# cassiePython/NeRF-Art

Hardware: AMD Instinct MI355X
Metric: rays/sec at 480x270x128spp VolSDF render (higher is better)
Workload: dtype pixels bf16x3 (sdf, nabla, radiance, compositing of the 192 final samples: f32 split into 2 bf16 terms, 3 MFMAs per product, f32 accumulate), Algorithm-1 sampler fp16x1 on error-compensated one-term weights (fp16 act x fp16 weight, 1 MFMA per product, f32 accumulate; model.calibrate_sampler()), guar

## Files before the change

### nerfart_amd/csrc/ray_common.h

```cpp
#pragma once
#include "nerfart_common.h"
#include "sample_cdf.h"
#include <math.h>

namespace nerfart {

__device__ __forceinline__ float wave_sum(float v) {
#pragma unroll
    for (int o = 32; o > 0; o >>= 1) v += __shfl_xor(v, o, 64);
    return v;
}
__device__ __forceinline__ float wave_max(float v) {
#pragma unroll
    for (int o = 32; o > 0; o >>= 1) v = fmaxf(v, __shfl_xor(v, o, 64));
    return v;
}
__device__ __forceinline__ float wave_excl_sum(float v) {
    const int lane = threadIdx.x & 63;
#pragma unroll
    for (int o = 1; o < 64; o <<= 1) {
        const float t = __shfl_up(v, o, 64);
        if (lane >= o) v += t;
    }
    const float e = __shfl_up(v, 1, 64);
// ... 82 lines not shown
            sR = __fmaf_rn(delta, sg, sR);
            sE = __fmaf_rn(t, x, sE);
        }
    }
    float R = wave_excl_sum(sR), E = wave_excl_sum(sE);
    float mx = -INFINITY;
#pragma unroll
    for (int i = 0; i < MAXSEG; ++i) {
        const int k = k0 + i;
        if (k < k1) {
            E = __fmaf_rn(c_t[i], c_x[i], E);
            float b = expf(-R) * (expf(E) - 1.f);
            if (isnan(b)) b = INFINITY;
            if (clamp) b = fminf(fmaxf(b, 0.f), 1e5f);
            if (w_out) w_out[k] = b;
            mx = fmaxf(mx, b);
            R = __fmaf_rn(c_delta[i], c_sigma[i], R);
        }
    }
    return wave_max(mx);
}

template <int MAXSEG>
struct SegConsts { float delta[MAXSEG], s[MAXSEG], dstar[MAXSEG], dd[MAXSEG]; int cnt; };

template <int MAXSEG>
__device__ __forceinline__ void load_seg_consts(const float* d, const float* s, int n, SegConsts<MAXSEG>& C) {
    const int lane = threadIdx.x & 63;
    const int nint = n - 1;
    const int seg = (nint + 63) >> 6;
    const int k0 = lane * seg;
    const int k1 = (k0 + seg < nint) ? k0 + seg : nint;
    C.cnt = k1 - k0;
    float dk = 0.f, sk = 0.f;
    if (k0 < k1) { dk = d[k0]; sk = s[k0]; }
#pragma unroll
    for (int i = 0; i < MAXSEG; ++i) {
        C.delta[i] = 0.f; C.s[i] = 0.f; C.dstar[i] = 0.f; C.dd[i] = 0.f;
        if (i < C.cnt) {
            const float dn = d[k0 + i + 1], sn = s[k0 + i + 1];
            const float delta = dn - dk;
            C.delta[i] = delta;
            C.s[i] = sk;
            C.dstar[i] = fmaxf(0.5f * (fabsf(sk) + fabsf(sn) - delta), 0.f);
            C.dd[i] = delta * delta;
            dk = dn; sk = sn;
        }
    }
}

template <int MAXSEG>
__device__ __forceinline__ float scan_consts(const SegConsts<MAXSEG>& C, float alpha, float beta) {
    const float a4b = alpha / (4.f * beta);
    float c_sigma[MAXSEG], c_t[MAXSEG], c_x[MAXSEG];
    float sR = 0.f, sE = 0.f;
#pragma unroll
    for (int i = 0; i < MAXSEG; ++i) {
        c_sigma[i] = 0.f; c_t[i] = 0.f; c_x[i] = 0.f;
        if (i < C.cnt) {
            const float sg = sdf_to_sigma(C.s[i], alpha, beta);
            const float t = a4b * C.dd[i];
            const float x = expf(-C.dstar[i] / beta);
            c_sigma[i] = sg; c_t[i] = t; c_x[i] = x;
            sR = __fmaf_rn(C.delta[i], sg, sR);
            sE = __fmaf_rn(t, x, sE);
        }
    }
    float R = wave_excl_sum(sR), E = wave_excl_sum(sE);
    float mx = -INFINITY;
#pragma unroll
    for (int i = 0; i < MAXSEG; ++i) {
        if (i < C.cnt) {
            E = __fmaf_rn(c_t[i], c_x[i], E);
            float b = expf(-R) * (expf(E) - 1.f);
            if (isnan(b)) b = INFINITY;
            mx = fmaxf(mx, b);
            R = __fmaf_rn(C.delta[i], c_sigma[i], R);
        }
    }
    return wave_max(mx);
}

__device__ __forceinline__ float error_bound_scan(const float* d, const float* s, int n, float alpha, float beta,
                                                  float* w_out, bool clamp) {
#ifndef NERFART_SCAN_GENERIC
    const int seg = (n - 1 + 63) >> 6;
    if (seg <= 8) return error_bound_scan_cached<8>(d, s, n, alpha, beta, w_out, clamp);
    if (seg <= 16) return error_bound_scan_cached<16>(d, s, n, alpha, beta, w_out, clamp);
    if (seg <= 24) return error_bound_scan_cached<24>(d, s, n, alpha, beta, w_out, clamp);
#endif
    return error_bound_scan_generic(d, s, n, alpha, beta, w_out, clamp);
}

__device__ __forceinline__ void opacity_cdf(const float* d, const float* s, int n, float alpha, float beta, float* cdf) {
    const int lane = threadIdx.x & 63;
    const int nint = n - 1;
    const int seg = (nint + 63) >> 6;
    const int k0 = lane * seg;
    const int k1 = (k0 + seg < nint) ? k0 + seg : nint;
    float sR = 0.f;
    for (int k = k0; k < k1; ++k) sR += sdf_to_sigma(s[k], alpha, beta) * (d[k + 1] - d[k]);
    float R = wave_excl_sum(sR);
    if (lane == 0) cdf[0] = 0.f;
    for (int k = k0; k < k1; ++k) {
        cdf[k + 1] = 1.f - expf(-R);
        R += sdf_to_sigma(s[k], alpha, beta) * (d[k + 1] - d[k]);
    }
}

__device__ __forceinline__ void bitonic_sort(float* a, int n) {
    const int lane = threadIdx.x & 63;
    for (int k = 2; k <= n; k <<= 1) {
        for (int j = k >> 1; j > 0; j >>= 1) {
            __syncthreads();
// ... 15 lines not shown
```

### nerfart_amd/csrc/volsdf_render.hip

```cpp
#include "ray_common.h"
#include "host_util.h"
#include <cstdlib>

namespace nerfart {

struct SamplerParams {
    int n;
    int cap;
    int n_up;
    int n_final;
    int max_bisect;
    int it;
    float eps;
    float alpha_net, beta_net;
    int u_final_stride;
    float guard;
    int* esc_list;
    int* esc_count;
};

__device__ __forceinline__ bool in_guard_band(const SamplerParams& P, float mx) {
    return P.guard > 0.f && fabsf(mx - P.eps) <= P.guard * P.eps;
}
__device__ __forceinline__ void escalate(const SamplerParams& P, int ray) {
// ... 8 lines not shown
    const int r = (int)(i / n), k = (int)(i - (long long)r * n);
    const float nr = near ? near[r] : near_s, fr = far ? far[r] : far_s;
    const float tk = t[k];
    out[(size_t)r * stride + k] = __fadd_rn(__fmul_rn(nr, __fsub_rn(1.f, tk)), __fmul_rn(fr, tk));
}

__global__ void k_normalize_dirs(const float* __restrict__ in, float* __restrict__ out, int n) {
    const int i = blockIdx.x * blockDim.x + threadIdx.x;
    if (i >= n) return;
    const float x = in[3 * i], y = in[3 * i + 1], z = in[3 * i + 2];
    const float nrm = fmaxf(sqrtf(x * x + y * y + z * z), 1e-12f);
    out[3 * i] = x / nrm; out[3 * i + 1] = y / nrm; out[3 * i + 2] = z / nrm;
}

__device__ __forceinline__ void load_row(float* dst, const float* src, int n) {
    for (int i = threadIdx.x; i < n; i += 64) dst[i] = src[i];
}

__device__ __forceinline__ void emit_final_samples(const float* d, const float* cdf, int n, const float* u_final,
                                                   int n_final, float* out) {
    for (int j = threadIdx.x; j < n_final; j += 64) out[j] = invert_cdf_at(d, cdf, n, u_final[j]);
}

__global__ void __launch_bounds__(64)
k_first_check(SamplerParams P, const float* __restrict__ dA, const float* __restrict__ sA,
              const float* __restrict__ u_final, float beta_plus0_denom, const float* __restrict__ far,
              float far_s, float* __restrict__ d_fine, float* __restrict__ beta_plus, float* __restrict__ beta_map,
              float* __restrict__ iter_usage, int* __restrict__ act_out, int* __restrict__ act_count) {
    extern __shared__ __attribute__((aligned(16))) float sm[];
    const int ray = blockIdx.x;
    float* d = sm; float* s = sm + P.n; float* cdf = sm + 2 * P.n;
    load_row(d, dA + (size_t)ray * P.cap, P.n);
    load_row(s, sA + (size_t)ray * P.cap, P.n);
    __syncthreads();
    const float mx = error_bound_scan(d, s, P.n, P.alpha_net, P.beta_net, nullptr, false);
    const float fr = far ? far[ray] : far_s;
    if (in_guard_band(P, mx)) { escalate(P, ray); return; }
    if (!(mx > P.eps)) {
        opacity_cdf(d, s, P.n, P.alpha_net, P.beta_net, cdf);
        __syncthreads();
        emit_final_samples(d, cdf, P.n, u_final + (size_t)ray * P.u_final_stride, P.n_final, d_fine + (size_t)ray * P.n_final);
        if (threadIdx.x == 0) { iter_usage[ray] = 0.f; beta_map[ray] = P.beta_net; }
    } else if (threadIdx.x == 0) {
        beta_plus[ray] = sqrtf((fr * fr) / beta_plus0_denom);
        act_out[atomicAdd(act_count, 1)] = ray;
    }
}

__global__ void __launch_bounds__(64)
k_upsample(SamplerParams P, const float* __restrict__ dA, const float* __restrict__ sA,
           const int* __restrict__ act, const float* __restrict__ beta_plus, const float* __restrict__ u_up,
           int clamp_bounds, int always_sort, float* __restrict__ d_new) {
    extern __shared__ __attribute__((aligned(16))) float sm[];
    const int slot = blockIdx.x, ray = act[slot];
    const int n = P.n;
    float* d = sm; float* s = sm + n; float* cdf = sm + 2 * n; float* w = sm + 3 * n; float* out = sm + 4 * n;
    load_row(d, dA + (size_t)ray * P.cap, n);
    load_row(s, sA + (size_t)ray * P.cap, n);
    __syncthreads();
    const float bp = beta_plus[ray];
    error_bound_scan(d, s, n, 1.f / bp, bp, w, clamp_bounds != 0);
    __syncthreads();
    const int lane = threadIdx.x;
    const int nint = n - 1, seg = (nint + 63) >> 6, k0 = lane * seg, k1 = (k0 + seg < nint) ? k0 + seg : nint;
    float part = 0.f;
    for (int k = k0; k < k1; ++k) { const float wk = w[k] + 1e-5f; w[k] = wk; part += wk; }
    const float total = wave_sum(part);
    float ps = 0.f;
    for (int k = k0; k < k1; ++k) ps += w[k] / total;
    float run = wave_excl_sum(ps);
    if (lane == 0) cdf[0] = 0.f;
    for (int k = k0; k < k1; ++k) { run += w[k] / total; cdf[k + 1] = run; }
    __syncthreads();
    for (int j = lane; j < P.n_up; j += 64) out[j] = invert_cdf_at(d, cdf, n, u_up[j + 1]);
    __syncthreads();
    if (always_sort || !__all((int)lane_row_in_order(out, P.n_up, lane))) bitonic_sort(out, P.n_up);
    for (int j = lane; j < P.n_up; j += 64) d_new[(size_t)slot * P.n_up + j] = out[j];
}

template <int MAXSEG>
__device__ __forceinline__ void merge_check_tail(const SamplerParams& P, int ray, const float* d, const float* s, float* cdf, int nm,
                                                 const float* __restrict__ u_final, float* __restrict__ d_fine, float* __restrict__ beta_plus,
                                                 float* __restrict__ beta_map, float* __restrict__ iter_usage, int* __restrict__ act_out,
                                                 int* __restrict__ act_count) {
    constexpr int NS = MAXSEG > 0 ? MAXSEG : 1;
    SegConsts<NS> C;
    if constexpr (MAXSEG > 0) load_seg_consts<NS>(d, s, nm, C);
    auto scan = [&](float alpha, float beta) -> float {
        if constexpr (MAXSEG > 0) return scan_consts<NS>(C, alpha, beta);
        else return error_bound_scan(d, s, nm, alpha, beta, nullptr, false);
    };
    const float mx = scan(P.alpha_net, P.beta_net);
    if (in_guard_band(P, mx)) { escalate(P, ray); return; }
    if (!(mx > P.eps)) {
        opacity_cdf(d, s, nm, P.alpha_net, P.beta_net, cdf);
        __syncthreads();
        emit_final_samples(d, cdf, nm, u_final + (size_t)ray * P.u_final_stride, P.n_final, d_fine + (size_t)ray * P.n_final);
        if (threadIdx.x == 0) { iter_usage[ray] = (float)P.it; beta_map[ray] = P.beta_net; }
    } else {
        float hi = beta_plus[ray], lo = P.beta_net;
        for (int b = 0; b < P.max_bisect; ++b) {
            const float mid = 0.5f * (lo + hi);
            const float m = scan(1.f / mid, mid);
            if (m <= P.eps) hi = mid; else lo = mid;
        }
        if (threadIdx.x == 0) {
            beta_plus[ray] = hi;
            act_out[atomicAdd(act_count, 1)] = ray;
        }
    }
}

__global__ void __launch_bounds__(64)
k_merge_check(SamplerParams P, const float* __restrict__ dA, const float* __restrict__ sA,
              float* __restrict__ dB, float* __restrict__ sB, const int* __restrict__ act,
              const float* __restrict__ d_new, const float* __restrict__ s_new, const float* __restrict__ u_final,
              float* __restrict__ d_fine, float* __restrict__ beta_plus, float* __restrict__ beta_map,
              float* __restrict__ iter_usage, int* __restrict__ act_out, int* __restrict__ act_count) {
    extern __shared__ __attribute__((aligned(16))) float sm[];
    const int slot = blockIdx.x, ray = act[slot];
    const int n = P.n, nu = P.n_up, nm = n + nu;
    float* d_old = sm; float* dn = sm + n;
    float* d = dn + nu; float* s = d + nm;
    const float* s_old = sA + (size_t)ray * P.cap;
    const float* sn = s_new + (size_t)slot * nu;
    load_row(d_old, dA + (size_t)ray * P.cap, n);
    load_row(dn, d_new + (size_t)slot * nu, nu);
    __syncthreads();
    for (int i = threadIdx.x; i < n; i += 64) {
        const int r = i + lower_bound(dn, nu, d_old[i]);
        d[r] = d_old[i]; s[r] = s_old[i];
    }
    for (int k = threadIdx.x; k < nu; k += 64) {
        const int r = k + upper_bound(d_old, n, dn[k]);
        d[r] = dn[k]; s[r] = sn[k];
    }
    __syncthreads();
    for (int i = threadIdx.x; i < nm; i += 64) {
        dB[(size_t)ray * P.cap + i] = d[i];
        sB[(size_t)ray * P.cap + i] = s[i];
    }
#ifndef NERFART_SCAN_GENERIC
    const int seg = (nm - 1 + 63) >> 6;
    if (seg <= 16) { merge_check_tail<16>(P, ray, d, s, d_old, nm, u_final, d_fine, beta_plus, beta_map, iter_usage, act_out, act_count); return; }
    if (seg <= 24) { merge_check_tail<24>(P, ray, d, s, d_old, nm, u_final, d_fine, beta_plus, beta_map, iter_usage, act_out, act_count); return; }
#endif
    merge_check_tail<0>(P, ray, d, s, d_old, nm, u_final, d_fine, beta_plus, beta_map, iter_usage, act_out, act_count);
}

__global__ void __launch_bounds__(64)
k_finalize_unconverged(SamplerParams P, const float* __restrict__ dA, const float* __restrict__ sA,
                       const int* __restrict__ act, const float* __restrict__ u_final,
                       const float* __restrict__ beta_plus, float* __restrict__ d_fine,
                       float* __restrict__ beta_map, float* __restrict__ iter_usage) {
    extern __shared__ __attribute__((aligned(16))) float sm[];
    const int ray = act[blockIdx.x];
    const int n = P.n;
    float* d = sm; float* s = sm + n; float* cdf = sm + 2 * n;
    load_row(d, dA + (size_t)ray * P.cap, n);
    load_row(s, sA + (size_t)ray * P.cap, n);
    __syncthreads();
    const float bp = beta_plus[ray];
    opacity_cdf(d, s, n, 1.f / bp, bp, cdf);
    __syncthreads();
    emit_final_samples(d, cdf, n, u_final + (size_t)ray * P.u_final_stride, P.n_final, d_fine + (size_t)ray * P.n_final);
    if (threadIdx.x == 0) { iter_usage[ray] = -1.f; beta_map[ray] = bp; }
}

__global__ void __launch_bounds__(64)
k_sort_concat(const float* __restrict__ a, int na, int a_stride, const float* __restrict__ b, int nb, int b_stride,
// ... 85 lines not shown
                                  float* __restrict__ beta_map, float* __restrict__ iter_usage) {
    const int slot = blockIdx.x, ray = list[slot], t = threadIdx.x;
    if (slot >= n) return;
    for (int j = t; j < n_final; j += 64) d_fine[(size_t)ray * n_final + j] = c_d_fine[(size_t)slot * n_final + j];
    if (t == 0) { beta_map[ray] = c_beta[slot]; iter_usage[ray] = c_iter[slot]; }
}

enum { SKIP_SEG = 32 };
constexpr float SKIP_THETA = 128.0f;

__global__ void k_live_init(int c0, int n, int* __restrict__ live, float* __restrict__ osum) {
    const int i = blockIdx.x * blockDim.x + threadIdx.x;
    if (i < n) { live[i] = c0 + i; osum[c0 + i] = 0.f; }
}

__global__ void k_gather_segment_depths(const int* __restrict__ live, int n_live, int P, int e0, int len, const float* __restrict__ d_all,
                                        float* __restrict__ c_d) {
    const long long i = (long long)blockIdx.x * blockDim.x + threadIdx.x;
    if (i >= (long long)n_live * len) return;
    const int slot = (int)(i / len), j = (int)(i - (long long)slot * len);
    c_d[i] = d_all[(size_t)live[slot] * P + e0 + j];
}

__global__ void k_scatter_segment(const int* __restrict__ live, int n_live, int P, int e0, int len, const float* __restrict__ c_sdf,
                                  const float* __restrict__ c_nabla, const float* __restrict__ c_rad, float* __restrict__ sdf,
                                  float* __restrict__ nabla, float* __restrict__ rad) {
    const long long i = (long long)blockIdx.x * blockDim.x + threadIdx.x;
    if (i >= (long long)n_live * len) return;
    const int slot = (int)(i / len), j = (int)(i - (long long)slot * len);
    const size_t q = (size_t)live[slot] * P + e0 + j;
    sdf[q] = c_sdf[i];
#pragma unroll
    for (int c = 0; c < 3; ++c) { nabla[3 * q + c] = c_nabla[3 * (size_t)i + c]; rad[3 * q + c] = c_rad[3 * (size_t)i + c]; }
}

__global__ void __launch_bounds__(256)
k_advance_live(const int* __restrict__ live, int n_live, int P, int e0, int len, const float* __restrict__ d_all, float alpha, float beta,
               float* __restrict__ osum, int* __restrict__ alive, float* sdf, float* __restrict__ nabla, float* __restrict__ rad) {
    const int slot = blockIdx.x * 4 + (threadIdx.x >> 6), lane = threadIdx.x & 63;
    if (slot >= n_live) return;
    const int ray = live[slot];
    const float* dr = d_all + (size_t)ray * P;
    const float* sr = sdf + (size_t)ray * P;
    float x = 0.f;
    if (lane < len) {
        const int k = e0 + lane;
        x = fmaxf(sdf_to_sigma(sr[k], alpha, beta) * (dr[k + 1] - dr[k]), 0.f);
    }
    float sum = osum[ray];
    for (int j = 0; j < len; ++j) sum = __fadd_rn(sum, __shfl(x, j, 64));
    const bool dead = sum >= SKIP_THETA;
    if (lane == 0) { osum[ray] = sum; alive[slot] = dead ? 0 : 1; }
    if (dead) {
        const size_t q0 = (size_t)ray * P + e0 + len;
        const int n = P - (e0 + len);
        for (int i = lane; i < n; i += 64) sdf[q0 + i] = 0.f;
        for (int i = lane; i < 3 * n; i += 64) { nabla[3 * q0 + i] = 0.f; rad[3 * q0 + i] = 0.f; }
    }
}

__global__ void __launch_bounds__(1024)
k_compact_live(const int* __restrict__ live, const int* __restrict__ alive, int n_live, int* __restrict__ live_next, int* __restrict__ n_next) {
    __shared__ int wsum[16];
    __shared__ int base_sh;
    const int t = threadIdx.x, lane = t & 63, wv = t >> 6;
    const int first = blockIdx.x * 1024;
    int part = 0;
    for (int i = t; i < first; i += 1024) part += alive[i];
#pragma unroll
    for (int o = 32; o > 0; o >>= 1) part += __shfl_xor(part, o, 64);
    if (lane == 0) wsum[wv] = part;
    __syncthreads();
    if (t == 0) { int b = 0; for (int w = 0; w < 16; ++w) b += wsum[w]; base_sh = b; }
    __syncthreads();
    const int base = base_sh;
    const int slot = first + t;
    const bool keep = slot < n_live && alive[slot] != 0;
// ... 37 lines not shown
    NERFART_HIP(hipGetLastError());
    return 0;
}

static int check_rows(const char* who, int n, int cap, int n_extra) {
    char msg[160];
    if (n < 2 || n > cap) snprintf(msg, sizeof(msg), "%s: needs 2 <= n <= cap (n = %d, cap = %d)", who, n, cap);
    else if ((long long)n + n_extra > cap) snprintf(msg, sizeof(msg), "%s: n + n_up = %lld exceeds the row capacity cap = %d", who, (long long)n + n_extra, cap);
    else return 0;
    set_last_error(msg);
    return 2;
}

static const char kLdsRefusal[] = "per-ray kernel needs more than 160 KiB of LDS (too many samples per ray)";

static int first_check_launch(int n_rays, int n, int cap, int n_final, float eps, float alpha_net, float beta_net,
                              const float* dA, const float* sA, const float* u_final, int u_final_stride,
                              float beta_plus0_denom, const float* far, float far_s, float* d_fine, float* beta_plus,
                              float* beta_map, float* iter_usage, int* act_out, int* act_count, float guard, int* esc_list, int* esc_count,
                              void* stream) {
    if (n_rays <= 0) return 0;
    SamplerParams P{n, cap, 0, n_final, 0, 0, eps, alpha_net, beta_net, u_final_stride, guard, esc_list, esc_count};
    const size_t lds = (size_t)3 * n * sizeof(float);
    if (int rc = set_lds((const void*)k_first_check, lds, kLdsRefusal)) return rc;
    hipLaunchKernelGGL(k_first_check, dim3(n_rays), dim3(64), lds, (hipStream_t)stream, P, dA, sA, u_final,
                       beta_plus0_denom, far, far_s, d_fine, beta_plus, beta_map, iter_usage, act_out, act_count);
    NERFART_HIP(hipGetLastError());
    return 0;
}

int nerfart_volsdf_first_check(int n_rays, int n, int cap, int n_final, float eps, float alpha_net, float beta_net,
                               const float* dA, const float* sA, const float* u_final, int u_final_stride,
                               float beta_plus0_denom, const float* far, float far_s, float* d_fine, float* beta_plus,
                               float* beta_map, float* iter_usage, int* act_out, int* act_count, void* stream) {
    if (n_rays <= 0) return 0;
    if (int rc = check_rows("volsdf_first_check", n, cap, 0)) return rc;
    return first_check_launch(n_rays, n, cap, n_final, eps, alpha_net, beta_net, dA, sA, u_final, u_final_stride, beta_plus0_denom, far, far_s, d_fine,
                              beta_plus, beta_map, iter_usage, act_out, act_count, 0.f, nullptr, nullptr, stream);
}

static int upsample_launch(int n_active, int n, int cap, int n_up, const float* dA, const float* sA, const int* act,
                           const float* beta_plus, const float* u_up, int clamp_bounds, float* d_new, void* stream) {
    if (n_active <= 0) return 0;
    if (n_up & (n_up - 1)) { set_last_error("n_up must be a power of two"); return 2; }
    SamplerParams P{n, cap, n_up, 0, 0, 0, 0.f, 0.f, 0.f};
    const size_t lds = ((size_t)4 * n + n_up) * sizeof(float);
    if (int rc = set_lds((const void*)k_upsample, lds, kLdsRefusal)) return rc;
    const char* e = std::getenv("NERFART_UPSAMPLE_SORT");
    const int always_sort = (e != nullptr && e[0] == 'a') ? 1 : 0;
    hipLaunchKernelGGL(k_upsample, dim3(n_active), dim3(64), lds, (hipStream_t)stream, P, dA, sA, act, beta_plus, u_up,
                       clamp_bounds, always_sort, d_new);
    NERFART_HIP(hipGetLastError());
    return 0;
}

int nerfart_volsdf_upsample(int n_active, int n, int cap, int n_up, const float* dA, const float* sA, const int* act,
                            const float* beta_plus, const float* u_up, int clamp_bounds, float* d_new, void* stream) {
    if (n_active <= 0) return 0;
    if (int rc = check_rows("volsdf_upsample", n, cap, 0)) return rc;
    return upsample_launch(n_active, n, cap, n_up, dA, sA, act, beta_plus, u_up, clamp_bounds, d_new, stream);
}

static int merge_check_launch(int n_active, int n, int cap, int n_up, int n_final, int max_bisect, int it, float eps,
                              float alpha_net, float beta_net, const float* dA, const float* sA, float* dB, float* sB,
                              const int* act, const float* d_new, const float* s_new, const float* u_final,
                              int u_final_stride, float* d_fine, float* beta_plus, float* beta_map, float* iter_usage,
                              int* act_out, int* act_count, float guard, int* esc_list, int* esc_count, void* stream) {
    if (n_active <= 0) return 0;
    SamplerParams P{n, cap, n_up, n_final, max_bisect, it, eps, alpha_net, beta_net, u_final_stride, guard, esc_list, esc_count};
    const size_t lds = ((size_t)3 * n + 3 * n_up) * sizeof(float);
    if (int rc = set_lds((const void*)k_merge_check, lds, kLdsRefusal)) return rc;
    hipLaunchKernelGGL(k_merge_check, dim3(n_active), dim3(64), lds, (hipStream_t)stream, P, dA, sA, dB, sB, act, d_new,
                       s_new, u_final, d_fine, beta_plus, beta_map, iter_usage, act_out, act_count);
    NERFART_HIP(hipGetLastError());
    return 0;
}

int nerfart_volsdf_merge_check(int n_active, int n, int cap, int n_up, int n_final, int max_bisect, int it, float eps,
                               float alpha_net, float beta_net, const float* dA, const float* sA, float* dB, float* sB,
                               const int* act, const float* d_new, const float* s_new, const float* u_final,
                               int u_final_stride, float* d_fine, float* beta_plus, float* beta_map, float* iter_usage,
                               int* act_out, int* act_count, void* stream) {
    if (n_active <= 0) return 0;
    if (int rc = check_rows("volsdf_merge_check", n, cap, n_up)) return rc;
    return merge_check_launch(n_active, n, cap, n_up, n_final, max_bisect, it, eps, alpha_net, beta_net, dA, sA, dB, sB, act, d_new, s_new, u_final,
                              u_final_stride, d_fine, beta_plus, beta_map, iter_usage, act_out, act_count, 0.f, nullptr, nullptr, stream);
}

static int finalize_launch(int n_active, int n, int cap, int n_final, const float* dA, const float* sA, const int* act,
                           const float* u_final, int u_final_stride, const float* beta_plus, float* d_fine,
                           float* beta_map, float* iter_usage, void* stream) {
    if (n_active <= 0) return 0;
    SamplerParams P{n, cap, 0, n_final, 0, 0, 0.f, 0.f, 0.f, u_final_stride};
    const size_t lds = (size_t)3 * n * sizeof(float);
    if (int rc = set_lds((const void*)k_finalize_unconverged, lds, kLdsRefusal)) return rc;
// ... 105 lines not shown
    if (!own_tables) {
        w.t_init = const_cast<float*>(t_init_dev); w.u_up = const_cast<float*>(u_up_dev); w.u_final = const_cast<float*>(u_final_dev);
    } else {
        if (int rc = upload_linspace_tables({{w.t_init, n_init}, {w.u_up, n_up + 2}, {w.u_final, n_final}}, stream)) return rc;
        if (u_final_per_ray) w.u_final = const_cast<float*>(u_final_dev);
    }
    if (int rc = nerfart_linspace_depths(w.t_init, n_init, near, far, near_s, far_s, n_rays, w.dA, cap, stream)) return rc;
    if (int rc = nerfart_sdf_fwd_rays(surf_blob, precision, rays_o, rays_dn, nullptr, w.dA, n_rays, n_init, cap, R_bg, w.sA, cap, stream)) return rc;
    NERFART_HIP(hipMemsetAsync(w.count, 0, COUNT_SLOTS * sizeof(int), stream));
    const float denom = (float)(4.0 * (double)(n_init - 1) * log(1.0 + (double)eps));
    if (int rc = first_check_launch(n_rays, n_init, cap, n_final, eps, alpha_net, beta_net, w.dA, w.sA, w.u_final,
                                    u_stride, denom, far, far_s, d_fine, w.beta_plus, beta_map, iter_usage, w.act0,
                                    w.count, guard, w.esc_list, w.count + ESC_SLOT, stream)) return rc;
    int h_count[COUNT_SLOTS];
    NERFART_HIP(hipMemcpyAsync(h_count, w.count, sizeof(h_count), hipMemcpyDeviceToHost, stream));
    NERFART_HIP(hipStreamSynchronize(stream));
    int n_act = h_count[0];
    float *dA = w.dA, *sA = w.sA, *dB = w.dB, *sB = w.sB;
    int *act = w.act0, *act_next = w.act1;
    int n = n_init;
    for (int it = 1; it <= max_iter && n_act > 0; ++it) {
        if (int rc = upsample_launch(n_act, n, cap, n_up, dA, sA, act, w.beta_plus, w.u_up, it > 1, w.d_new, stream)) return rc;
        if (int rc = nerfart_sdf_fwd_rays(surf_blob, precision, rays_o, rays_dn, act, w.d_new, n_act, n_up, n_up, R_bg, w.s_new, n_up, stream)) return rc;
        if (int rc = merge_check_launch(n_act, n, cap, n_up, n_final, max_bisect, it, eps, alpha_net, beta_net, dA, sA,
                                        dB, sB, act, w.d_new, w.s_new, w.u_final, u_stride, d_fine, w.beta_plus,
                                        beta_map, iter_usage, act_next, w.count + it, guard, w.esc_list, w.count + ESC_SLOT, stream)) return rc;
        NERFART_HIP(hipMemcpyAsync(h_count, w.count, sizeof(h_count), hipMemcpyDeviceToHost, stream));
        NERFART_HIP(hipStreamSynchronize(stream));
        n_act = h_count[it];
        float* t;
        t = dA; dA = dB; dB = t;
        t = sA; sA = sB; sB = t;
        int* ti = act; act = act_next; act_next = ti;
        n += n_up;
        if (guarded && late_round > 0 && it >= late_round) break;
    }
    if (!guarded) {
        if (n_act > 0)
            if (int rc = finalize_launch(n_act, n, cap, n_final, dA, sA, act, w.u_final, u_stride, w.beta_plus, d_fine,
                                         beta_map, iter_usage, stream)) return rc;
        return 0;
    }
    int n_esc = h_count[ESC_SLOT];
    if (n_act > 0) {
        NERFART_HIP(hipMemcpyAsync(w.esc_list + n_esc, act, sizeof(int) * (size_t)n_act, hipMemcpyDeviceToDevice, stream));
        n_esc += n_act;
    }
    if (n_escalated) *n_escalated = n_esc;
    if (n_esc == 0) return 0;
    hipLaunchKernelGGL(k_gather_rays, dim3(n_esc), dim3(64), 0, stream, w.esc_list, n_esc, rays_o, rays_dn, near, far,
                       u_final_per_ray ? u_final_dev : (const float*)nullptr, n_final, w.c_o, w.c_dn, w.c_near, w.c_far, w.c_u);
    NERFART_HIP(hipGetLastError());
    const float* u2 = u_final_per_ray ? w.c_u : (own_tables ? nullptr : u_final_dev);
    const int* esc_list = w.esc_list;
    float *c_d_fine = w.c_d_fine, *c_beta = w.c_beta, *c_iter = w.c_iter;
    profile_class0_as(4);
    const int rc_esc = fine_sample_run(esc_blob, esc_precision, nullptr, 0, 0.f, 0, w.c_o, w.c_dn, n_esc, near ? w.c_near : nullptr, far ? w.c_far : nullptr,
                                       near_s, far_s, R_bg, alpha_net, beta_net, eps, n_init, n_up, n_final, max_iter, max_bisect,
// ... 32 lines not shown

int nerfart_volsdf_fine_sample_guarded(const float* surf_blob, int precision, const float* esc_blob, int esc_precision, float guard,
                                       const float* rays_o, const float* rays_dn, int n_rays,
                                       const float* near, const float* far, float near_s, float far_s, float R_bg,
                                       float alpha_net, float beta_net, float eps, int n_init, int n_up, int n_final,
                                       int max_iter, int max_bisect, const float* t_init_dev, const float* u_up_dev,
                                       const float* u_final_dev, int u_final_per_ray, float* d_fine, float* beta_map,
                                       float* iter_usage, int* n_escalated, void* workspace, long long workspace_bytes, void* stream) {
    return nerfart_volsdf_fine_sample_guarded2(surf_blob, precision, esc_blob, esc_precision, guard, 0, rays_o, rays_dn, n_rays, near, far, near_s, far_s, R_bg,
                                               alpha_net, beta_net, eps, n_init, n_up, n_final, max_iter, max_bisect, t_init_dev, u_up_dev, u_final_dev,
                                               u_final_per_ray, d_fine, beta_map, iter_usage, n_escalated, workspace, workspace_bytes, stream);
}

typedef struct {
    float *rays_dn, *d_fine, *d_coarse, *t_coarse, *d_all, *sdf, *nabla, *rad, *beta_map, *iter_usage, *h7;
    char* sampler;
    size_t sampler_bytes;
    char* nabla_ws;
    size_t nabla_ws_bytes;
} render_ws_t;

typedef struct {
    int *live0, *live1, *alive, *n_live;
    float *osum, *c_depth, *c_sdf, *c_nabla, *c_rad;
} skip_ws_t;

static skip_ws_t carve_skip(Carver& c, int R, int P, int G) {
    skip_ws_t k;
    const size_t gpts = (size_t)G * (P < SKIP_SEG ? P : SKIP_SEG);
    k.live0 = c.take<int>((size_t)G);
    k.live1 = c.take<int>((size_t)G);
    k.alive = c.take<int>((size_t)G);
    k.n_live = c.take<int>(1);
    k.osum = c.take<float>((size_t)R);
    k.c_depth = c.take<float>(gpts);
    k.c_sdf = c.take<float>(gpts);
    k.c_nabla = c.take<float>(gpts * 3);
    k.c_rad = c.take<float>(gpts * 3);
    return k;
}

static int skip_group_rays(int R, int P, int k3_rays, size_t room) {
    const long long rk = k3_rays < R ? k3_rays : R;
    long long g = rk * P / (P < SKIP_SEG ? P : SKIP_SEG);
    if (g > R) g = R;
    for (; g > 1; g /= 2) {
        Carver c(nullptr);
        carve_skip(c, R, P, (int)g);
        if (c.off <= room) break;
    }
    return (int)g;
}

static render_ws_t carve_render(Carver& c, int R, int n_samples, int n_imp, int max_iter, int k3_rays) {
    render_ws_t w;
    const int P = n_samples + n_imp;
    const int n_init = 4 * n_samples, n_up = 4 * n_samples;
    w.rays_dn = c.take<float>((size_t)R * 3);
    w.d_fine = c.take<float>((size_t)R * n_imp);
    w.d_coarse = c.take<float>((size_t)R * n_samples);
    w.t_coarse = c.take<float>((size_t)n_samples);
    w.d_all = c.take<float>((size_t)R * P);
    w.sdf = c.take<float>((size_t)R * P);
    w.nabla = c.take<float>((size_t)R * P * 3);
    w.rad = c.take<float>((size_t)R * P * 3);
    w.beta_map = c.take<float>((size_t)R);
    w.iter_usage = c.take<float>((size_t)R);
    const int rk = k3_rays < R ? k3_rays : R;
    w.h7 = c.take<float>((size_t)rk * P * 256);
    w.sampler_bytes = sampler_bytes(R, n_init + max_iter * n_up, n_up, n_init, n_imp);
    w.sampler = c.take<char>(w.sampler_bytes);
    const long long nb0 = nerfart_sdf_nabla_workspace_bytes(0), nb1 = nerfart_sdf_nabla_workspace_bytes(1);
    w.nabla_ws_bytes = (size_t)(nb0 > nb1 ? nb0 : nb1);
    w.nabla_ws = c.take<char>(w.nabla_ws_bytes);
    return w;
}

long long nerfart_volsdf_render_workspace_bytes(int n_rays, int n_samples, int n_importance, int max_upsample_steps,
                                                int k3_rays_chunk) {
    Carver c(nullptr);
    carve_render(c, n_rays, n_samples, n_importance, max_upsample_steps, k3_rays_chunk);
    return (long long)c.off;
}

static int final_stage_skipping(const render_ws_t& w, const float* surf_blob, int precision, const float* rad_blob, int rad_precision, int view_tiles,
                                const float* rays_o, int n_rays, int P, float R_bg, float alpha, float beta, const float* d_all, float* sdf,
                                float* nabla, float* rad, int k3_rays, hipStream_t stream) {
    const int G = skip_group_rays(n_rays, P, k3_rays, w.sampler_bytes);
    Carver carver(w.sampler);
    const skip_ws_t k = carve_skip(carver, n_rays, P, G);
    if (carver.off > w.sampler_bytes) { set_last_error("render: workspace too small"); return 2; }
    int *live = k.live0, *live_next = k.live1;
    for (int c0 = 0; c0 < n_rays; c0 += G) {
        int n_live = (n_rays - c0 < G) ? n_rays - c0 : G;
        hipLaunchKernelGGL(k_live_init, dim3((n_live + 255) / 256), dim3(256), 0, stream, c0, n_live, live, k.osum);
        NERFART_HIP(hipGetLastError());
        for (int e0 = 0; e0 < P && n_live > 0; e0 += SKIP_SEG) {
            const int len = (P - e0 < SKIP_SEG) ? P - e0 : SKIP_SEG;
            const unsigned nb = (unsigned)(((long long)n_live * len + 255) / 256);
            hipLaunchKernelGGL(k_gather_segment_depths, dim3(nb), dim3(256), 0, stream, live, n_live, P, e0, len, d_all, k.c_depth);
            NERFART_HIP(hipGetLastError());
            if (int rc = nerfart_sdf_nabla_fwd_rays(surf_blob, precision, rays_o, w.rays_dn, live, k.c_depth, n_live, len, len, R_bg, k.c_sdf, k.c_nabla,
                                                    w.h7, w.nabla_ws, (long long)w.nabla_ws_bytes, stream)) return rc;
            if (int rc = nerfart_radiance_fwd_rays(rad_blob, rad_precision, view_tiles, rays_o, w.rays_dn, live, k.c_depth, n_live, len, len, k.c_nabla,
                                                   w.h7, k.c_rad, stream)) return rc;
            hipLaunchKernelGGL(k_scatter_segment, dim3(nb), dim3(256), 0, stream, live, n_live, P, e0, len, k.c_sdf, k.c_nabla, k.c_rad, sdf, nabla, rad);
            NERFART_HIP(hipGetLastError());
            if (e0 + len >= P) break;
            hipLaunchKernelGGL(k_advance_live, dim3((n_live + 3) / 4), dim3(256), 0, stream, live, n_live, P, e0, len, d_all, alpha, beta, k.osum,
                               k.alive, sdf, nabla, rad);
            NERFART_HIP(hipGetLastError());
            hipLaunchKernelGGL(k_compact_live, dim3((n_live + 1023) / 1024), dim3(1024), 0, stream, live, k.alive, n_live, live_next, k.n_live);
            NERFART_HIP(hipGetLastError());
            NERFART_HIP(hipMemcpyAsync(&n_live, k.n_live, sizeof(int), hipMemcpyDeviceToHost, stream));
            NERFART_HIP(hipStreamSynchronize(stream));
            int* t = live; live = live_next; live_next = t;
        }
    }
    return 0;
}

int nerfart_volsdf_render_staged2_fwd(const float* surf_blob, int precision, const float* rad_blob, int rad_precision, const float* sampler_blob,
                                     int sampler_precision, float sampler_guard, int sampler_late_round, int view_tiles, const float* rays_o,
                              const float* rays_d, int n_rays, float near_s, float far_s, float R_bg, float alpha,
                              float beta, float eps, int n_samples, int n_importance, int max_upsample_steps,
                              int max_bisection_steps, int white_bkgd, int k3_rays_chunk, const float* t_coarse_dev,
                              const float* t_init_dev, const float* u_up_dev, const float* u_final_dev, int u_final_per_ray,
                              float* rgb, float* depth, float* acc, float* normals, float* d_all_out, float* sdf_out, float* nabla_out,
                              float* radiance_out, float* sigma_out, float* p_out, float* tau_out, float* beta_map_out,
                              float* iter_usage_out, int* n_escalated, void* workspace, long long workspace_bytes, void* stream_) {
    hipStream_t stream = (hipStream_t)stream_;
    if (n_rays <= 0) return 0;
    if (!sampler_blob) { set_last_error("render: sampler_blob is NULL"); return 2; }
    if (n_samples < 2 || n_importance < 1 || k3_rays_chunk < 1) { set_last_error("render: bad sample counts"); return 2; }
// ... 89 lines not shown
```

Before: 344,200.

## Specialize sampler scans at launch, trim LDS rows, fuse scatter/advance, own h7 scratch

```diff
diff --git a/nerfart_amd/csrc/ray_common.h b/nerfart_amd/csrc/ray_common.h
--- a/nerfart_amd/csrc/ray_common.h
+++ b/nerfart_amd/csrc/ray_common.h
@@ -128,7 +128,7 @@
 }
 
 template <int MAXSEG>
-struct SegConsts { float delta[MAXSEG], s[MAXSEG], dstar[MAXSEG], dd[MAXSEG]; int cnt; };
+struct SegConsts { float delta[MAXSEG], s[MAXSEG], dstar[MAXSEG]; int cnt; };
 
 template <int MAXSEG>
 __device__ __forceinline__ void load_seg_consts(const float* d, const float* s, int n, SegConsts<MAXSEG>& C) {
@@ -142,32 +142,36 @@
     if (k0 < k1) { dk = d[k0]; sk = s[k0]; }
 #pragma unroll
     for (int i = 0; i < MAXSEG; ++i) {
-        C.delta[i] = 0.f; C.s[i] = 0.f; C.dstar[i] = 0.f; C.dd[i] = 0.f;
+        C.delta[i] = 0.f; C.s[i] = 0.f; C.dstar[i] = 0.f;
         if (i < C.cnt) {
             const float dn = d[k0 + i + 1], sn = s[k0 + i + 1];
             const float delta = dn - dk;
             C.delta[i] = delta;
             C.s[i] = sk;
             C.dstar[i] = fmaxf(0.5f * (fabsf(sk) + fabsf(sn) - delta), 0.f);
-            C.dd[i] = delta * delta;
             dk = dn; sk = sn;
         }
     }
+}
+
+__device__ __forceinline__ float squared_here(float v) {
+    asm volatile("" : "+v"(v));
+    return v * v;
 }
 
 template <int MAXSEG>
 __device__ __forceinline__ float scan_consts(const SegConsts<MAXSEG>& C, float alpha, float beta) {
     const float a4b = alpha / (4.f * beta);
-    float c_sigma[MAXSEG], c_t[MAXSEG], c_x[MAXSEG];
+    float c_sigma[MAXSEG], c_x[MAXSEG];
     float sR = 0.f, sE = 0.f;
 #pragma unroll
     for (int i = 0; i < MAXSEG; ++i) {
-        c_sigma[i] = 0.f; c_t[i] = 0.f; c_x[i] = 0.f;
+        c_sigma[i] = 0.f; c_x[i] = 0.f;
         if (i < C.cnt) {
             const float sg = sdf_to_sigma(C.s[i], alpha, beta);
-            const float t = a4b * C.dd[i];
+            const float t = a4b * squared_here(C.delta[i]);
             const float x = expf(-C.dstar[i] / beta);
-            c_sigma[i] = sg; c_t[i] = t; c_x[i] = x;
+            c_sigma[i] = sg; c_x[i] = x;
             sR = __fmaf_rn(C.delta[i], sg, sR);
             sE = __fmaf_rn(t, x, sE);
         }
@@ -177,7 +181,7 @@
 #pragma unroll
     for (int i = 0; i < MAXSEG; ++i) {
         if (i < C.cnt) {
-            E = __fmaf_rn(c_t[i], c_x[i], E);
+            E = __fmaf_rn(a4b * squared_here(C.delta[i]), c_x[i], E);
             float b = expf(-R) * (expf(E) - 1.f);
             if (isnan(b)) b = INFINITY;
             mx = fmaxf(mx, b);
@@ -187,15 +191,22 @@
     return wave_max(mx);
 }
 
+inline int scan_maxseg(int n) {
+#ifndef NERFART_SCAN_GENERIC
+    const int seg = (n - 1 + 63) >> 6;
+    if (seg <= 8) return 8;
+    if (seg <= 16) return 16;
+    if (seg <= 24) return 24;
+#endif
+    (void)n;
+    return 0;
+}
+
+template <int MAXSEG>
 __device__ __forceinline__ float error_bound_scan(const float* d, const float* s, int n, float alpha, float beta,
                                                   float* w_out, bool clamp) {
-#ifndef NERFART_SCAN_GENERIC
-    const int seg = (n - 1 + 63) >> 6;
-    if (seg <= 8) return error_bound_scan_cached<8>(d, s, n, alpha, beta, w_out, clamp);
-    if (seg <= 16) return error_bound_scan_cached<16>(d, s, n, alpha, beta, w_out, clamp);
-    if (seg <= 24) return error_bound_scan_cached<24>(d, s, n, alpha, beta, w_out, clamp);
-#endif
-    return error_bound_scan_generic(d, s, n, alpha, beta, w_out, clamp);
+    if constexpr (MAXSEG > 0) return error_bound_scan_cached<MAXSEG>(d, s, n, alpha, beta, w_out, clamp);
+    else return error_bound_scan_generic(d, s, n, alpha, beta, w_out, clamp);
 }
 
 __device__ __forceinline__ void opacity_cdf(const float* d, const float* s, int n, float alpha, float beta, float* cdf) {
diff --git a/nerfart_amd/csrc/volsdf_render.hip b/nerfart_amd/csrc/volsdf_render.hip
--- a/nerfart_amd/csrc/volsdf_render.hip
+++ b/nerfart_amd/csrc/volsdf_render.hip
@@ -54,6 +54,7 @@
     for (int j = threadIdx.x; j < n_final; j += 64) out[j] = invert_cdf_at(d, cdf, n, u_final[j]);
 }
 
+template <int MAXSEG>
 __global__ void __launch_bounds__(64)
 k_first_check(SamplerParams P, const float* __restrict__ dA, const float* __restrict__ sA,
               const float* __restrict__ u_final, float beta_plus0_denom, const float* __restrict__ far,
@@ -65,7 +66,7 @@
     load_row(d, dA + (size_t)ray * P.cap, P.n);
     load_row(s, sA + (size_t)ray * P.cap, P.n);
     __syncthreads();
-    const float mx = error_bound_scan(d, s, P.n, P.alpha_net, P.beta_net, nullptr, false);
+    const float mx = error_bound_scan<MAXSEG>(d, s, P.n, P.alpha_net, P.beta_net, nullptr, false);
     const float fr = far ? far[ray] : far_s;
     if (in_guard_band(P, mx)) { escalate(P, ray); return; }
     if (!(mx > P.eps)) {
@@ -79,6 +80,7 @@
     }
 }
 
+template <int MAXSEG, bool S_IN_LDS>
 __global__ void __launch_bounds__(64)
 k_upsample(SamplerParams P, const float* __restrict__ dA, const float* __restrict__ sA,
            const int* __restrict__ act, const float* __restrict__ beta_plus, const float* __restrict__ u_up,
@@ -86,12 +88,13 @@
     extern __shared__ __attribute__((aligned(16))) float sm[];
     const int slot = blockIdx.x, ray = act[slot];
     const int n = P.n;
-    float* d = sm; float* s = sm + n; float* cdf = sm + 2 * n; float* w = sm + 3 * n; float* out = sm + 4 * n;
+    float* d = sm; float* cdf = sm + n; float* w = sm + 2 * n; float* out = sm + 3 * n;
+    const float* s = sA + (size_t)ray * P.cap;
     load_row(d, dA + (size_t)ray * P.cap, n);
-    load_row(s, sA + (size_t)ray * P.cap, n);
+    if constexpr (S_IN_LDS) { float* sl = out + P.n_up; load_row(sl, s, n); s = sl; }
     __syncthreads();
     const float bp = beta_plus[ray];
-    error_bound_scan(d, s, n, 1.f / bp, bp, w, clamp_bounds != 0);
+    error_bound_scan<MAXSEG>(d, s, n, 1.f / bp, bp, w, clamp_bounds != 0);
     __syncthreads();
     const int lane = threadIdx.x;
     const int nint = n - 1, seg = (nint + 63) >> 6, k0 = lane * seg, k1 = (k0 + seg < nint) ? k0 + seg : nint;
@@ -110,24 +113,33 @@
     for (int j = lane; j < P.n_up; j += 64) d_new[(size_t)slot * P.n_up + j] = out[j];
 }
 
-template <int MAXSEG>
-__device__ __forceinline__ void merge_check_tail(const SamplerParams& P, int ray, const float* d, const float* s, float* cdf, int nm,
+template <int MAXSEG, bool ROWS_IN_LDS>
+__device__ __forceinline__ void merge_check_tail(const SamplerParams& P, int ray, const float* d, const float* s, float* r0, float* r1, int nm,
                                                  const float* __restrict__ u_final, float* __restrict__ d_fine, float* __restrict__ beta_plus,
                                                  float* __restrict__ beta_map, float* __restrict__ iter_usage, int* __restrict__ act_out,
                                                  int* __restrict__ act_count) {
     constexpr int NS = MAXSEG > 0 ? MAXSEG : 1;
+    const float *dl = d, *sl = s;
+    if constexpr (!ROWS_IN_LDS) { load_row(r0, d, nm); load_row(r1, s, nm); __syncthreads(); dl = r0; sl = r1; }
     SegConsts<NS> C;
-    if constexpr (MAXSEG > 0) load_seg_consts<NS>(d, s, nm, C);
+    if constexpr (MAXSEG > 0) load_seg_consts<NS>(dl, sl, nm, C);
     auto scan = [&](float alpha, float beta) -> float {
         if constexpr (MAXSEG > 0) return scan_consts<NS>(C, alpha, beta);
-        else return error_bound_scan(d, s, nm, alpha, beta, nullptr, false);
+        else return error_bound_scan<0>(dl, sl, nm, alpha, beta, nullptr, false);
     };
     const float mx = scan(P.alpha_net, P.beta_net);
     if (in_guard_band(P, mx)) { escalate(P, ray); return; }
     if (!(mx > P.eps)) {
-        opacity_cdf(d, s, nm, P.alpha_net, P.beta_net, cdf);
-        __syncthreads();
-        emit_final_samples(d, cdf, nm, u_final + (size_t)ray * P.u_final_stride, P.n_final, d_fine + (size_t)ray * P.n_final);
+        if constexpr (ROWS_IN_LDS) {
+            opacity_cdf(d, s, nm, P.alpha_net, P.beta_net, r0);
+            __syncthreads();
+            emit_final_samples(d, r0, nm, u_final + (size_t)ray * P.u_final_stride, P.n_final, d_fine + (size_t)ray * P.n_final);
+        } else {
+            __syncthreads();
+            opacity_cdf(r0, s, nm, P.alpha_net, P.beta_net, r1);
+            __syncthreads();
+            emit_final_samples(r0, r1, nm, u_final + (size_t)ray * P.u_final_stride, P.n_final, d_fine + (size_t)ray * P.n_final);
+        }
         if (threadIdx.x == 0) { iter_usage[ray] = (float)P.it; beta_map[ray] = P.beta_net; }
     } else {
         float hi = beta_plus[ray], lo = P.beta_net;
@@ -143,17 +155,20 @@
     }
 }
 
+template <int MAXSEG, bool ROWS_IN_LDS>
 __global__ void __launch_bounds__(64)
-k_merge_check(SamplerParams P, const float* __restrict__ dA, const float* __restrict__ sA,
-              float* __restrict__ dB, float* __restrict__ sB, const int* __restrict__ act,
-              const float* __restrict__ d_new, const float* __restrict__ s_new, const float* __restrict__ u_final,
-              float* __restrict__ d_fine, float* __restrict__ beta_plus, float* __restrict__ beta_map,
-              float* __restrict__ iter_usage, int* __restrict__ act_out, int* __restrict__ act_count) {
+k_merge_check(SamplerParams P, const float* __restrict__ dA, const float* __restrict__ sA, float* dB, float* sB, const int* __restrict__ act,
+              const float* __restrict__ d_new, const float* __restrict__ s_new, const float* __restrict__ u_final, float* __restrict__ d_fine,
+              float* __restrict__ beta_plus, float* __restrict__ beta_map, float* __restrict__ iter_usage, int* __restrict__ act_out,
+              int* __restrict__ act_count) {
     extern __shared__ __attribute__((aligned(16))) float sm[];
     const int slot = blockIdx.x, ray = act[slot];
     const int n = P.n, nu = P.n_up, nm = n + nu;
     float* d_old = sm; float* dn = sm + n;
-    float* d = dn + nu; float* s = d + nm;
+    float* row1 = dn + nu;
+    float* dg = dB + (size_t)ray * P.cap; float* sg = sB + (size_t)ray * P.cap;
+    float* d = ROWS_IN_LDS ? row1 : dg;
+    float* s = ROWS_IN_LDS ? row1 + nm : sg;
     const float* s_old = sA + (size_t)ray * P.cap;
     const float* sn = s_new + (size_t)slot * nu;
     load_row(d_old, dA + (size_t)ray * P.cap, n);
@@ -167,17 +182,12 @@
         const int r = k + upper_bound(d_old, n, dn[k]);
         d[r] = dn[k]; s[r] = sn[k];
     }
-    __syncthreads();
-    for (int i = threadIdx.x; i < nm; i += 64) {
-        dB[(size_t)ray * P.cap + i] = d[i];
-        sB[(size_t)ray * P.cap + i] = s[i];
-    }
-#ifndef NERFART_SCAN_GENERIC
-    const int seg = (nm - 1 + 63) >> 6;
-    if (seg <= 16) { merge_check_tail<16>(P, ray, d, s, d_old, nm, u_final, d_fine, beta_plus, beta_map, iter_usage, act_out, act_count); return; }
-    if (seg <= 24) { merge_check_tail<24>(P, ray, d, s, d_old, nm, u_final, d_fine, beta_plus, beta_map, iter_usage, act_out, act_count); return; }
-#endif
-    merge_check_tail<0>(P, ray, d, s, d_old, nm, u_final, d_fine, beta_plus, beta_map, iter_usage, act_out, act_count);
+    if constexpr (!ROWS_IN_LDS) __threadfence_block();
+    __syncthreads();
+    if constexpr (ROWS_IN_LDS) {
+        for (int i = threadIdx.x; i < nm; i += 64) { dg[i] = d[i]; sg[i] = s[i]; }
+    }
+    merge_check_tail<MAXSEG, ROWS_IN_LDS>(P, ray, d, s, d_old, row1, nm, u_final, d_fine, beta_plus, beta_map, iter_usage, act_out, act_count);
 }
 
 __global__ void __launch_bounds__(64)
@@ -309,37 +319,30 @@
     c_d[i] = d_all[(size_t)live[slot] * P + e0 + j];
 }
 
-__global__ void k_scatter_segment(const int* __restrict__ live, int n_live, int P, int e0, int len, const float* __restrict__ c_sdf,
-                                  const float* __restrict__ c_nabla, const float* __restrict__ c_rad, float* __restrict__ sdf,
-                                  float* __restrict__ nabla, float* __restrict__ rad) {
-    const long long i = (long long)blockIdx.x * blockDim.x + threadIdx.x;
-    if (i >= (long long)n_live * len) return;
-    const int slot = (int)(i / len), j = (int)(i - (long long)slot * len);
-    const size_t q = (size_t)live[slot] * P + e0 + j;
-    sdf[q] = c_sdf[i];
-#pragma unroll
-    for (int c = 0; c < 3; ++c) { nabla[3 * q + c] = c_nabla[3 * (size_t)i + c]; rad[3 * q + c] = c_rad[3 * (size_t)i + c]; }
-}
-
 __global__ void __launch_bounds__(256)
-k_advance_live(const int* __restrict__ live, int n_live, int P, int e0, int len, const float* __restrict__ d_all, float alpha, float beta,
-               float* __restrict__ osum, int* __restrict__ alive, float* sdf, float* __restrict__ nabla, float* __restrict__ rad) {
+k_scatter_advance(const int* __restrict__ live, int n_live, int P, int e0, int len, int advance, const float* __restrict__ c_sdf,
+                  const float* __restrict__ c_nabla, const float* __restrict__ c_rad, const float* __restrict__ d_all, float alpha, float beta,
+                  float* __restrict__ osum, int* __restrict__ alive, float* __restrict__ sdf, float* __restrict__ nabla, float* __restrict__ rad) {
     const int slot = blockIdx.x * 4 + (threadIdx.x >> 6), lane = threadIdx.x & 63;
     if (slot >= n_live) return;
     const int ray = live[slot];
+    const size_t c0 = (size_t)slot * len, q = (size_t)ray * P + e0;
+    float sk = 0.f;
+    if (lane < len) { sk = c_sdf[c0 + lane]; sdf[q + lane] = sk; }
+    for (int i = lane; i < 3 * len; i += 64) { nabla[3 * q + i] = c_nabla[3 * c0 + i]; rad[3 * q + i] = c_rad[3 * c0 + i]; }
+    if (!advance) return;
     const float* dr = d_all + (size_t)ray * P;
-    const float* sr = sdf + (size_t)ray * P;
     float x = 0.f;
     if (lane < len) {
         const int k = e0 + lane;
-        x = fmaxf(sdf_to_sigma(sr[k], alpha, beta) * (dr[k + 1] - dr[k]), 0.f);
+        x = fmaxf(sdf_to_sigma(sk, alpha, beta) * (dr[k + 1] - dr[k]), 0.f);
     }
     float sum = osum[ray];
     for (int j = 0; j < len; ++j) sum = __fadd_rn(sum, __shfl(x, j, 64));
     const bool dead = sum >= SKIP_THETA;
     if (lane == 0) { osum[ray] = sum; alive[slot] = dead ? 0 : 1; }
     if (dead) {
-        const size_t q0 = (size_t)ray * P + e0 + len;
+        const size_t q0 = q + len;
         const int n = P - (e0 + len);
         for (int i = lane; i < n; i += 64) sdf[q0 + i] = 0.f;
         for (int i = lane; i < 3 * n; i += 64) { nabla[3 * q0 + i] = 0.f; rad[3 * q0 + i] = 0.f; }
@@ -423,8 +426,10 @@
     if (n_rays <= 0) return 0;
     SamplerParams P{n, cap, 0, n_final, 0, 0, eps, alpha_net, beta_net, u_final_stride, guard, esc_list, esc_count};
     const size_t lds = (size_t)3 * n * sizeof(float);
-    if (int rc = set_lds((const void*)k_first_check, lds, kLdsRefusal)) return rc;
-    hipLaunchKernelGGL(k_first_check, dim3(n_rays), dim3(64), lds, (hipStream_t)stream, P, dA, sA, u_final,
+    const int m = scan_maxseg(n);
+    auto* const kernel = m == 8 ? k_first_check<8> : m == 16 ? k_first_check<16> : m == 24 ? k_first_check<24> : k_first_check<0>;
+    if (int rc = set_lds((const void*)kernel, lds, kLdsRefusal)) return rc;
+    hipLaunchKernelGGL(kernel, dim3(n_rays), dim3(64), lds, (hipStream_t)stream, P, dA, sA, u_final,
                        beta_plus0_denom, far, far_s, d_fine, beta_plus, beta_map, iter_usage, act_out, act_count);
     NERFART_HIP(hipGetLastError());
     return 0;
@@ -440,16 +445,33 @@
                               beta_plus, beta_map, iter_usage, act_out, act_count, 0.f, nullptr, nullptr, stream);
 }
 
+static bool perray_lds_ref() {
+    const char* e = std::getenv("NERFART_PERRAY_LDS");
+    return e != nullptr && e[0] == 'r';
+}
+
+typedef void (*upsample_fn)(SamplerParams, const float*, const float*, const int*, const float*, const float*, int, int, float*);
+static upsample_fn upsample_kernel(int maxseg, bool ref) {
+    switch (maxseg) {
+    case 8: return ref ? k_upsample<8, true> : k_upsample<8, false>;
+    case 16: return ref ? k_upsample<16, true> : k_upsample<16, false>;
+    case 24: return ref ? k_upsample<24, true> : k_upsample<24, false>;
+    default: return ref ? k_upsample<0, true> : k_upsample<0, false>;
+    }
+}
+
 static int upsample_launch(int n_active, int n, int cap, int n_up, const float* dA, const float* sA, const int* act,
                            const float* beta_plus, const float* u_up, int clamp_bounds, float* d_new, void* stream) {
     if (n_active <= 0) return 0;
     if (n_up & (n_up - 1)) { set_last_error("n_up must be a power of two"); return 2; }
     SamplerParams P{n, cap, n_up, 0, 0, 0, 0.f, 0.f, 0.f};
-    const size_t lds = ((size_t)4 * n + n_up) * sizeof(float);
-    if (int rc = set_lds((const void*)k_upsample, lds, kLdsRefusal)) return rc;
+    const bool ref = perray_lds_ref();
+    const size_t lds = ((size_t)(ref ? 4 : 3) * n + n_up) * sizeof(float);
+    const upsample_fn kernel = upsample_kernel(scan_maxseg(n), ref);
+    if (int rc = set_lds((const void*)kernel, lds, kLdsRefusal)) return rc;
     const char* e = std::getenv("NERFART_UPSAMPLE_SORT");
     const int always_sort = (e != nullptr && e[0] == 'a') ? 1 : 0;
-    hipLaunchKernelGGL(k_upsample, dim3(n_active), dim3(64), lds, (hipStream_t)stream, P, dA, sA, act, beta_plus, u_up,
+    hipLaunchKernelGGL(kernel, dim3(n_active), dim3(64), lds, (hipStream_t)stream, P, dA, sA, act, beta_plus, u_up,
                        clamp_bounds, always_sort, d_new);
     NERFART_HIP(hipGetLastError());
     return 0;
@@ -460,6 +482,15 @@
     if (n_active <= 0) return 0;
     if (int rc = check_rows("volsdf_upsample", n, cap, 0)) return rc;
     return upsample_launch(n_active, n, cap, n_up, dA, sA, act, beta_plus, u_up, clamp_bounds, d_new, stream);
+}
+
+typedef void (*merge_check_fn)(SamplerParams, const float*, const float*, float*, float*, const int*, const float*, const float*, const float*, float*,
+                               float*, float*, float*, int*, int*);
+static merge_check_fn merge_check_kernel(int nm, bool ref) {
+    const int m = scan_maxseg(nm);
+    if (m == 8 || m == 16) return ref ? k_merge_check<16, true> : k_merge_check<16, false>;
+    if (m == 24) return ref ? k_merge_check<24, true> : k_merge_check<24, false>;
+    return ref ? k_merge_check<0, true> : k_merge_check<0, false>;
 }
 
 static int merge_check_launch(int n_active, int n, int cap, int n_up, int n_final, int max_bisect, int it, float eps,
@@ -469,9 +500,11 @@
                               int* act_out, int* act_count, float guard, int* esc_list, int* esc_count, void* stream) {
     if (n_active <= 0) return 0;
     SamplerParams P{n, cap, n_up, n_final, max_bisect, it, eps, alpha_net, beta_net, u_final_stride, guard, esc_list, esc_count};
-    const size_t lds = ((size_t)3 * n + 3 * n_up) * sizeof(float);
-    if (int rc = set_lds((const void*)k_merge_check, lds, kLdsRefusal)) return rc;
-    hipLaunchKernelGGL(k_merge_check, dim3(n_active), dim3(64), lds, (hipStream_t)stream, P, dA, sA, dB, sB, act, d_new,
+    const bool ref = perray_lds_ref();
+    const merge_check_fn kernel = merge_check_kernel(n + n_up, ref);
+    const size_t lds = (size_t)(ref ? 3 : 2) * ((size_t)n + n_up) * sizeof(float);
+    if (int rc = set_lds((const void*)kernel, lds, kLdsRefusal)) return rc;
+    hipLaunchKernelGGL(kernel, dim3(n_active), dim3(64), lds, (hipStream_t)stream, P, dA, sA, dB, sB, act, d_new,
                        s_new, u_final, d_fine, beta_plus, beta_map, iter_usage, act_out, act_count);
     NERFART_HIP(hipGetLastError());
     return 0;
@@ -623,7 +656,8 @@
     for (int it = 1; it <= max_iter && n_act > 0; ++it) {
         if (int rc = upsample_launch(n_act, n, cap, n_up, dA, sA, act, w.beta_plus, w.u_up, it > 1, w.d_new, stream)) return rc;
         if (int rc = nerfart_sdf_fwd_rays(surf_blob, precision, rays_o, rays_dn, act, w.d_new, n_act, n_up, n_up, R_bg, w.s_new, n_up, stream)) return rc;
-        if (int rc = merge_check_launch(n_act, n, cap, n_up, n_final, max_bisect, it, eps, alpha_net, beta_net, dA, sA,
+        const bool last_round = guarded && (it == max_iter || (late_round > 0 && it >= late_round));
+        if (int rc = merge_check_launch(n_act, n, cap, n_up, n_final, last_round ? 0 : max_bisect, it, eps, alpha_net, beta_net, dA, sA,
                                         dB, sB, act, w.d_new, w.s_new, w.u_final, u_stride, d_fine, w.beta_plus,
                                         beta_map, iter_usage, act_next, w.count + it, guard, w.esc_list, w.count + ESC_SLOT, stream)) return rc;
         NERFART_HIP(hipMemcpyAsync(h_count, w.count, sizeof(h_count), hipMemcpyDeviceToHost, stream));
@@ -634,7 +668,7 @@
         t = sA; sA = sB; sB = t;
         int* ti = act; act = act_next; act_next = ti;
         n += n_up;
-        if (guarded && late_round > 0 && it >= late_round) break;
+        if (last_round) break;
     }
     if (!guarded) {
         if (n_act > 0)
@@ -713,10 +747,10 @@
 
 typedef struct {
     int *live0, *live1, *alive, *n_live;
-    float *osum, *c_depth, *c_sdf, *c_nabla, *c_rad;
+    float *osum, *c_depth, *c_sdf, *c_nabla, *c_rad, *h7;
 } skip_ws_t;
 
-static skip_ws_t carve_skip(Carver& c, int R, int P, int G) {
+static skip_ws_t carve_skip(Carver& c, int R, int P, int G, bool own_h7) {
     skip_ws_t k;
     const size_t gpts = (size_t)G * (P < SKIP_SEG ? P : SKIP_SEG);
     k.live0 = c.take<int>((size_t)G);
@@ -728,18 +762,25 @@
     k.c_sdf = c.take<float>(gpts);
     k.c_nabla = c.take<float>(gpts * 3);
     k.c_rad = c.take<float>(gpts * 3);
+    k.h7 = own_h7 ? c.take<float>(gpts * 256) : nullptr;
     return k;
 }
 
-static int skip_group_rays(int R, int P, int k3_rays, size_t room) {
+static int skip_group_rays(int R, int P, int k3_rays, size_t room, bool* own_h7) {
     const long long rk = k3_rays < R ? k3_rays : R;
-    long long g = rk * P / (P < SKIP_SEG ? P : SKIP_SEG);
-    if (g > R) g = R;
-    for (; g > 1; g /= 2) {
+    long long g_shared = rk * P / (P < SKIP_SEG ? P : SKIP_SEG);
+    if (g_shared > R) g_shared = R;
+    const auto fits = [&](long long g, bool own) {
         Carver c(nullptr);
-        carve_skip(c, R, P, (int)g);
-        if (c.off <= room) break;
-    }
+        carve_skip(c, R, P, (int)g, own);
+        return c.off <= room;
+    };
+    *own_h7 = true;
+    for (long long g = R; g > g_shared; g /= 2)
+        if (fits(g, true)) return (int)g;
+    *own_h7 = false;
+    long long g = g_shared;
+    for (; g > 1 && !fits(g, false); g /= 2) {}
     return (int)g;
 }
 
@@ -777,10 +818,12 @@
 static int final_stage_skipping(const render_ws_t& w, const float* surf_blob, int precision, const float* rad_blob, int rad_precision, int view_tiles,
                                 const float* rays_o, int n_rays, int P, float R_bg, float alpha, float beta, const float* d_all, float* sdf,
                                 float* nabla, float* rad, int k3_rays, hipStream_t stream) {
-    const int G = skip_group_rays(n_rays, P, k3_rays, w.sampler_bytes);
+    bool own_h7 = false;
+    const int G = skip_group_rays(n_rays, P, k3_rays, w.sampler_bytes, &own_h7);
     Carver carver(w.sampler);
-    const skip_ws_t k = carve_skip(carver, n_rays, P, G);
+    const skip_ws_t k = carve_skip(carver, n_rays, P, G, own_h7);
     if (carver.off > w.sampler_bytes) { set_last_error("render: workspace too small"); return 2; }
+    float* h7 = own_h7 ? k.h7 : w.h7;
     int *live = k.live0, *live_next = k.live1;
     for (int c0 = 0; c0 < n_rays; c0 += G) {
         int n_live = (n_rays - c0 < G) ? n_rays - c0 : G;
@@ -792,15 +835,14 @@
             hipLaunchKernelGGL(k_gather_segment_depths, dim3(nb), dim3(256), 0, stream, live, n_live, P, e0, len, d_all, k.c_depth);
             NERFART_HIP(hipGetLastError());
             if (int rc = nerfart_sdf_nabla_fwd_rays(surf_blob, precision, rays_o, w.rays_dn, live, k.c_depth, n_live, len, len, R_bg, k.c_sdf, k.c_nabla,
-                                                    w.h7, w.nabla_ws, (long long)w.nabla_ws_bytes, stream)) return rc;
+                                                    h7, w.nabla_ws, (long long)w.nabla_ws_bytes, stream)) return rc;
             if (int rc = nerfart_radiance_fwd_rays(rad_blob, rad_precision, view_tiles, rays_o, w.rays_dn, live, k.c_depth, n_live, len, len, k.c_nabla,
-                                                   w.h7, k.c_rad, stream)) return rc;
-            hipLaunchKernelGGL(k_scatter_segment, dim3(nb), dim3(256), 0, stream, live, n_live, P, e0, len, k.c_sdf, k.c_nabla, k.c_rad, sdf, nabla, rad);
+                                                   h7, k.c_rad, stream)) return rc;
+            const bool last = e0 + len >= P;
+            hipLaunchKernelGGL(k_scatter_advance, dim3((n_live + 3) / 4), dim3(256), 0, stream, live, n_live, P, e0, len, last ? 0 : 1, k.c_sdf, k.c_nabla,
+                               k.c_rad, d_all, alpha, beta, k.osum, k.alive, sdf, nabla, rad);
             NERFART_HIP(hipGetLastError());
-            if (e0 + len >= P) break;
-            hipLaunchKernelGGL(k_advance_live, dim3((n_live + 3) / 4), dim3(256), 0, stream, live, n_live, P, e0, len, d_all, alpha, beta, k.osum,
-                               k.alive, sdf, nabla, rad);
-            NERFART_HIP(hipGetLastError());
+            if (last) break;
             hipLaunchKernelGGL(k_compact_live, dim3((n_live + 1023) / 1024), dim3(1024), 0, stream, live, k.alive, n_live, live_next, k.n_live);
             NERFART_HIP(hipGetLastError());
             NERFART_HIP(hipMemcpyAsync(&n_live, k.n_live, sizeof(int), hipMemcpyDeviceToHost, stream));
```

Measured after the change: 352,700, median of 6. 2.5% higher.
